# zju3dv/LoG

Measured on AMD Instinct MI355X. Metric: Gaussians/sec fwd+bwd @1080p, higher is better.
Workload: dtype f32; 1 GPU; 30M random Gaussians (seed 0, opacity 0.999), 1920x1080, 8 orbit views/GPU, fwd+bwd; north_star / configs[3] per GPU; gaussians=30000000, width=1920, height=1080, views_per_gpu=8, streams_per_gpu=1, parallelism=single GPU, 1 view(s) in flight per GPU (HIP streams)

## Files before the change

include/lograst.h:

```cpp
#ifndef LOGRAST_H
#define LOGRAST_H

#include <stddef.h>
#include <stdint.h>

#ifdef __cplusplus
extern "C" {
#endif

#define LOGRAST_VERSION 4
#define LOGRAST_TILE 16
#define LOGRAST_REC_FLOATS 16
#define LOGRAST_BWD_ROW_FLOATS 16

#define LOGRAST_FILTER_NONE 0
#define LOGRAST_FORM_AUTO 0
#define LOGRAST_FORM_ROWS 1
#define LOGRAST_FORM_QUADRANT 2
#define LOGRAST_FILTER_DILATE 1
#define LOGRAST_FILTER_CLAMP 2

#define LOGRAST_STATUS_WORDS 8
#define LOGRAST_STATUS_OVERFLOW 0
#define LOGRAST_STATUS_LAST_INSTANCES 1
// ... 102 lines not shown

size_t lograst_sparse_segment_floats(int32_t kmax);
int lograst_pack_rows(const float* rows, int32_t groups, int64_t rows_per_group, int32_t kmax, float* packed,
                      uint32_t* overflow, void* stream);
int lograst_pack_rows_clear(float* rows, int32_t groups, int64_t rows_per_group, int32_t kmax, float* packed,
                            uint32_t* overflow, void* stream);
int lograst_pack_rows_hinted(float* rows, int32_t groups, int64_t rows_per_group, int32_t kmax, float* packed,
                             uint32_t* overflow, int32_t clear, const uint32_t* hint, int64_t hint_rows, void* stream);
int lograst_unpack_rows(float* dest, const float* packed, int32_t segments, int32_t kmax, int64_t rows_per_group,
                        int64_t dest_group_rows, int32_t atomic, void* stream);
int lograst_add_visible(float* seen, const int32_t* radii, int64_t n, void* stream);
int lograst_add_visible_n(float* seen, const int32_t* const* radii, int32_t k, int64_t n, void* stream);

int lograst_knob_count(void);
int lograst_knob_info(int32_t index, const char** name, int32_t* dflt, int32_t* lo, int32_t* hi, const char** what);
int lograst_set_knob(const char* name, int32_t value);
int lograst_get_knob(const char* name, int32_t* value);
int lograst_reset_knobs(void);

int lograst_read_state(const void* tile_state, uint32_t* num_instances_host, uint32_t* overflow_host,
                       uint32_t* max_tile_len_host, uint32_t* rect_instances_host, void* stream);

int lograst_set_tile_cull(int enabled);

#define LOGRAST_BWD_SCRATCH_ZEROED 1
#define LOGRAST_BWD_ACCUMULATE 2
#define LOGRAST_BWD_CONIC_TOUCHED_ONLY 4
#define LOGRAST_BWD_ACCUMULATE_ROWS 8
#define LOGRAST_GRAD_ROW_FLOATS 16

int lograst_backward(const lograst_view* view, int32_t n, const float* means3d, const float* scales,
                     const float* rotations, const int32_t* radii, const void* geom, const void* tile_state,
                     const uint32_t* point_list, const float* final_t, const int32_t* n_contrib,
                     const float* dl_dimage, float* dl_dmeans2d, float* bwd_rows, float* dl_dopacities,
                     float* dl_dcolors, float* dl_dmeans3d, float* dl_dscales, float* dl_drotations,
                     const float* point_weight, int32_t flags, void* stream);

int lograst_backward_aux(const lograst_view* view, int32_t n, const float* means3d, const float* scales,
                         const float* rotations, const int32_t* radii, const void* geom, const void* tile_state,
                         const uint32_t* point_list, const float* final_t, const int32_t* n_contrib,
                         const float* aux_colors, const float* dl_dimage, const float* dl_daux_image, float* dl_dmeans2d,
                         float* bwd_rows, int32_t bwd_row_floats, float* dl_dopacities, float* dl_dcolors,
                         float* dl_daux_colors, float* dl_dmeans3d, float* dl_dscales, float* dl_drotations,
                         const float* point_weight, int32_t flags, void* stream);

int lograst_project_backward(const lograst_view* view, int32_t n, const float* means3d, const float* scales,
// ... 314 lines not shown
```

log_amd/_lib.py:

```python
import ctypes
import os

_HERE = os.path.dirname(os.path.abspath(__file__))
LIB_PATH = os.environ.get("LOGRAST_LIB") or os.path.join(_HERE, "lib", "liblograst.so")

FILTER_NONE, FILTER_DILATE, FILTER_CLAMP = 0, 1, 2
FORM_AUTO, FORM_ROWS, FORM_QUADRANT = 0, 1, 2
GRAD_ROW_FLOATS = 16
REC_FLOATS = 16
BWD_ROW_FLOATS = 16
NUM_KERNELS = 22
NUM_KERNEL_SLOTS = 23

c_void_p, c_int32, c_uint32, c_float, c_size_t = (ctypes.c_void_p, ctypes.c_int32, ctypes.c_uint32,
                                                  ctypes.c_float, ctypes.c_size_t)


class LograstView(ctypes.Structure):
    _fields_ = [
        ("width", c_int32), ("height", c_int32),
        ("tanfovx", c_float), ("tanfovy", c_float),
        ("scale_modifier", c_float),
        ("filter_mode", c_int32), ("ndc_cull", c_int32), ("extras", c_int32),
        ("viewmatrix", c_void_p), ("projmatrix", c_void_p), ("bg", c_void_p),
# ... 92 lines not shown
                            + [c_void_p] * 7 + [c_int32, c_void_p, c_void_p, c_void_p, c_void_p]),
    "lograst_forward_render_aux": (ctypes.c_int, [ctypes.POINTER(LograstView), c_int32, c_void_p, c_void_p, c_void_p,
                                                  c_void_p, c_uint32, c_uint32, c_void_p, c_void_p, c_void_p, c_void_p,
                                                  c_void_p, c_void_p, c_void_p, c_int32, c_void_p, c_void_p, c_void_p,
                                                  c_void_p]),
    "lograst_forward_speculative_aux": (ctypes.c_int, [ctypes.POINTER(LograstView), c_int32] + [c_void_p] * 10
                                        + [c_uint32, c_uint32] + [c_void_p] * 7 + [c_int32, c_void_p, c_void_p, c_void_p]
                                        + [ctypes.POINTER(c_uint32), ctypes.POINTER(c_uint32), c_void_p]),
    "lograst_tile_rows": (ctypes.c_int, [ctypes.POINTER(LograstView), c_int32, c_void_p, c_void_p, c_void_p, c_void_p,
                                         c_void_p]),
    "lograst_stream_copy": (ctypes.c_int, [c_void_p, c_void_p, c_size_t, c_int32, c_void_p]),
    "lograst_sparse_segment_floats": (c_size_t, [c_int32]),
    "lograst_pack_rows": (ctypes.c_int, [c_void_p, c_int32, ctypes.c_int64, c_int32, c_void_p, c_void_p, c_void_p]),
    "lograst_pack_rows_clear": (ctypes.c_int, [c_void_p, c_int32, ctypes.c_int64, c_int32, c_void_p, c_void_p, c_void_p]),
    "lograst_pack_rows_hinted": (ctypes.c_int, [c_void_p, c_int32, ctypes.c_int64, c_int32, c_void_p, c_void_p, c_int32, c_void_p,
                                                ctypes.c_int64, c_void_p]),
    "lograst_add_visible": (ctypes.c_int, [c_void_p, c_void_p, ctypes.c_int64, c_void_p]),
    "lograst_add_visible_n": (ctypes.c_int, [c_void_p, c_void_p, c_int32, ctypes.c_int64, c_void_p]),
    "lograst_unpack_rows": (ctypes.c_int, [c_void_p, c_void_p, c_int32, c_int32, ctypes.c_int64, ctypes.c_int64, c_int32,
                                           c_void_p]),
    "lograst_read_state": (ctypes.c_int, [c_void_p, ctypes.POINTER(c_uint32), ctypes.POINTER(c_uint32),
                                          ctypes.POINTER(c_uint32), ctypes.POINTER(c_uint32), c_void_p]),
    "lograst_set_tile_cull": (ctypes.c_int, [ctypes.c_int]),
    "lograst_knob_count": (ctypes.c_int, []),
    "lograst_knob_info": (ctypes.c_int, [c_int32, ctypes.POINTER(ctypes.c_char_p), ctypes.POINTER(c_int32),
                                         ctypes.POINTER(c_int32), ctypes.POINTER(c_int32), ctypes.POINTER(ctypes.c_char_p)]),
    "lograst_set_knob": (ctypes.c_int, [ctypes.c_char_p, c_int32]),
    "lograst_get_knob": (ctypes.c_int, [ctypes.c_char_p, ctypes.POINTER(c_int32)]),
    "lograst_reset_knobs": (ctypes.c_int, []),
    "lograst_backward": (ctypes.c_int, [ctypes.POINTER(LograstView), c_int32] + [c_void_p] * 18 + [c_int32, c_void_p]),
    "lograst_backward_aux": (ctypes.c_int, [ctypes.POINTER(LograstView), c_int32] + [c_void_p] * 14 + [c_int32]
                             + [c_void_p] * 7 + [c_int32, c_void_p]),
    "lograst_project_backward": (ctypes.c_int, [ctypes.POINTER(LograstView), c_int32] + [c_void_p] * 10),
    "lograst_camera_scratch_bytes": (c_size_t, [c_int32]),
    "lograst_backward_camera": (ctypes.c_int, [ctypes.POINTER(LograstView), c_int32] + [c_void_p] * 18 + [c_int32]
                                + [c_void_p] * 3 + [c_size_t, c_void_p]),
    "lograst_project_backward_camera": (ctypes.c_int, [ctypes.POINTER(LograstView), c_int32] + [c_void_p] * 12
                                        + [c_size_t, c_void_p]),
    "lograst_pose_apply": (ctypes.c_int, [c_int32, c_int32] + [c_void_p] * 7),
    "lograst_pose_backward": (ctypes.c_int, [c_int32, c_int32] + [c_void_p] * 8),
    "lograst_sh_forward": (ctypes.c_int, [c_int32, c_int32, c_int32] + [c_void_p] * 6),
    "lograst_sh_backward": (ctypes.c_int, [c_int32, c_int32, c_int32] + [c_void_p] * 7 + [c_int32, c_void_p]),
    "lograst_knn_scratch_bytes": (c_size_t, [c_int32]),
    "lograst_knn_mean_dist2": (ctypes.c_int, [c_int32, c_void_p, c_void_p, c_void_p, c_size_t, c_void_p]),
    "lograst_lod_scratch_bytes": (c_size_t, [c_int32, c_int32, c_int32]),
    "lograst_lod_traverse": (ctypes.c_int, [c_int32, c_int32, c_int32] + [c_void_p] * 6 + [c_int32, c_void_p, c_void_p,
# ... 125 lines not shown
```

log_amd/csrc/api.hip:

```cpp
#include <hip/hip_runtime.h>

#include <cmath>
#include <cstdint>
#include <cstdio>
#include <cstdlib>
#include <cstring>
#include <mutex>
#include <atomic>
#include <string>
#include <vector>

#include "common.hpp"
#include "launch.hpp"
#include "decide.hpp"

static thread_local std::string g_err;
static int lr_fail(int code, const std::string& msg) {
  g_err = msg;
  return code;
}
#define LR_HIP(expr)                                                                                   \
  do {                                                                                                 \
    hipError_t _e = (expr);                                                                            \
    if (_e != hipSuccess)                                                                              \
// ... 94 lines not shown
}
static bool lr_big_input(int32_t n) { return n >= lr_knob(LRKNOB_HELPER_MIN_N); }
static LrPlan lr_plan(const LrView& v, int32_t n) {
  LrPlan p;
  p.tiles = (uint32_t)v.gx * (uint32_t)v.gy;
  lr_pick_batch(p, n, (uint32_t)v.gx, (uint32_t)v.gy);
  p.batches = p.batch ? ((uint32_t)n + p.batch - 1u) / p.batch : 0u;
  p.band = lr_band_sparse(v, (int)p.batch);
  p.staged_k = lr_fill_staged_k(p);
  p.big_input = lr_big_input(n);
  return p;
}

static std::atomic<int> g_tile_cull{-1};
static int lr_tile_cull() {
  int c = g_tile_cull.load(std::memory_order_relaxed);
  if (c < 0) {
    c = lr_env_int("LOGRAST_TILE_CULL", 1) ? 1 : 0;
    g_tile_cull.store(c, std::memory_order_relaxed);
  }
  return c;
}

static const char* kKernelNames[LOGRAST_NUM_KERNELS] = {
    "compute_radius", "project", "scan_tiles", "fill_keys", "sort_small", "sort_large", "sort_huge",
    "blend_fwd", "blend_bwd", "project_bwd", "knn3", "lod_traverse", "counter_update", "sparse_adam",
    "id_histogram", "gather_activate", "activate_bwd", "count_huge", "rebase_slots", "lazy_tail",
    "loss_fwd", "loss_bwd", "recolor"};
struct ProfRec { int slot; hipEvent_t a, b; bool own_a; };
struct ProfLast { hipStream_t stream; unsigned long long call; hipEvent_t ev; bool valid; };
static thread_local unsigned long long g_prof_call = 0;
static ProfLast g_prof_last = {nullptr, 0, nullptr, false};
static bool g_prof_on = false;
static std::vector<ProfRec> g_prof_open;
static std::vector<ProfRec> g_prof_done;
static std::vector<hipEvent_t> g_event_pool;
static double g_prof_ms[LOGRAST_NUM_KERNELS];
static int64_t g_prof_cnt[LOGRAST_NUM_KERNELS];
static std::mutex g_prof_mu;

static hipEvent_t lr_get_event() {
  if (!g_event_pool.empty()) { hipEvent_t e = g_event_pool.back(); g_event_pool.pop_back(); return e; }
  hipEvent_t e;
  (void)hipEventCreate(&e);
  return e;
}
// ... 584 lines not shown
  if (value < k->lo || value > k->hi) return lr_fail(LOGRAST_ERR_ARG, std::string(name) + ": value out of range");
  std::lock_guard<std::mutex> lk(g_knob_mu);
  g_knob_set[k->id] = true;
  g_knob_over[k->id] = value;
  lr_resolve_knobs_locked();
  return LOGRAST_OK;
}
int lograst_get_knob(const char* name, int32_t* value) {
  const LrKnobInfo* k = lr_find_knob(name);
  if (!k || !value) return lr_fail(LOGRAST_ERR_ARG, "unknown knob or NULL pointer");
  *value = lr_knob(k->id);
  return LOGRAST_OK;
}
int lograst_reset_knobs(void) {
  std::lock_guard<std::mutex> lk(g_knob_mu);
  for (bool& set : g_knob_set) set = false;
  lr_resolve_knobs_locked();
  return LOGRAST_OK;
}

int lograst_set_tile_cull(int enabled) {
  const int old = lr_tile_cull();
  g_tile_cull.store(enabled ? 1 : 0, std::memory_order_relaxed);
  return old;
}

int lograst_read_state(const void* tile_state, uint32_t* num_instances_host, uint32_t* overflow_host,
                       uint32_t* max_tile_len_host, uint32_t* rect_instances_host, void* stream) {
  if (!tile_state) return lr_fail(LOGRAST_ERR_ARG, "tile_state is NULL");
  uint32_t hdr[8] = {0, 0, 0, 0, 0, 0, 0, 0};
  hipStream_t s = (hipStream_t)stream;
  LR_HIP(hipMemcpyAsync(hdr, tile_state, sizeof(hdr), hipMemcpyDeviceToHost, s));
  LR_HIP(hipStreamSynchronize(s));
  if (num_instances_host) *num_instances_host = hdr[LR_HDR_NUM];
  if (overflow_host) *overflow_host = hdr[LR_HDR_OVERFLOW];
  if (max_tile_len_host) *max_tile_len_host = hdr[LR_HDR_MAXLEN];
  if (rect_instances_host) *rect_instances_host = hdr[LR_HDR_RECT];
  return LOGRAST_OK;
}

struct LrBackwardAux { int on; const float* aux_colors; const float* dl_daux_image; int32_t bwd_row_floats; float* dl_daux_colors; };
struct LrBackwardCam { int on; float* dl_dview; float* dl_dproj; void* scratch; size_t scratch_bytes; };
static int lr_check_camera(const LrView& v, int32_t n, int32_t flags, const LrBackwardCam& cam, hipStream_t s, bool* done) {
  *done = false;
  if (!cam.dl_dview || !cam.dl_dproj) return lr_fail(LOGRAST_ERR_ARG, "dl_dviewmatrix / dl_dprojmatrix are NULL");
  if (flags & (LOGRAST_BWD_ACCUMULATE | LOGRAST_BWD_ACCUMULATE_ROWS))
// ... 1181 lines not shown
```

log_amd/csrc/blend.hip:

```cpp
#include "common.hpp"
#include "launch.hpp"
#define LR_LANDED(q0, q1, c, i)                                                                                  \
  asm volatile("" : "+v"((q0).x), "+v"((q0).y), "+v"((q0).z), "+v"((q0).w), "+v"((q1).x), "+v"((q1).y), "+v"((q1).z), \
               "+v"((q1).w), "+v"(c), "+v"(i))

LR_DEV uint32_t lr_tile_of_block(uint32_t b, uint32_t tiles, int gx, int gy, int mode,
                                 const uint32_t* __restrict__ state) {
  if (mode == 3) return b < tiles ? state[lr_order_off(tiles) + b] : 0xffffffffu;
  if (mode == 1) {
    uint32_t nper = (tiles + 7u) >> 3;
    uint32_t t = (b & 7u) * nper + (b >> 3);
    return t < tiles ? t : 0xffffffffu;
  }
  if (mode == 2) {
    uint32_t nsbx = ((uint32_t)gx + 3u) >> 2, nsby = ((uint32_t)gy + 3u) >> 2;
    uint32_t r = b >> 3, sb = (r >> 4) * 8u + (b & 7u), local = r & 15u;
    if (sb >= nsbx * nsby) return 0xffffffffu;
    uint32_t tx = (sb % nsbx) * 4u + (local & 3u), ty = (sb / nsbx) * 4u + (local >> 2);
    if (tx >= (uint32_t)gx || ty >= (uint32_t)gy) return 0xffffffffu;
    return ty * (uint32_t)gx + tx;
  }
  return b < tiles ? b : 0xffffffffu;
}
static inline __host__ __device__ uint32_t lr_blend_grid(uint32_t tiles, int gx, int gy, int mode) {
// ... 527 lines not shown
  return lr_bank_select<0xc>(a + lr_dpp_perm<0x140>(a), b + lr_dpp_perm<0x140>(b));
}
LR_DEV float lr_row_pair4(float p, float q) {
  return lr_bank_select<0xa>(p + lr_dpp_perm<0x141>(p), q + lr_dpp_perm<0x141>(q));
}
LR_DEV float lr_quad_total(float x) {
  x = x + lr_dpp_perm<0xB1>(x);
  return x + lr_dpp_perm<0x4E>(x);
}

LR_DEV void lr_atomic_add_noret(float* p, float x) {
  asm volatile("global_atomic_add_f32 %0, %1, off" : : "v"(p), "v"(x) : "memory");
}

LR_DEV uint32_t lr_take_bit(uint64_t& m) {
  const uint32_t j = min((uint32_t)(__ffsll((long long)m) - 1), 64u);
  m &= m - 1ull;
  return j;
}
LR_DEV uint64_t lr_row_mask(int row, uint64_t m0, uint64_t m1, uint64_t m2, uint64_t m3) {
  return row == 0 ? m0 : (row == 1 ? m1 : (row == 2 ? m2 : m3));
}

template <bool MASKS>
__global__ void __launch_bounds__(256)
lr_blend_bwd_rows_kernel(LrView v, const float4* __restrict__ geom, const uint32_t* __restrict__ state,
                         uint32_t tiles, const uint32_t* __restrict__ plist, uint32_t capacity,
                         const float* __restrict__ final_T, const int* __restrict__ n_contrib,
                         const float* __restrict__ dL_dimage, float* __restrict__ acc_rows,
                         int xcd_mode, int block_test, const uint64_t* __restrict__ masks) {
  __shared__ float4 lr_stage[4][65 * LR_RB_SLOT];
  if (lr_bail(state, capacity)) return;
  const uint32_t tile = lr_tile_of_block(blockIdx.x, tiles, v.gx, v.gy, xcd_mode, state);
  if (tile >= tiles) return;
  const uint32_t* offsets = state + lr_offsets_off(tiles);
  const uint32_t beg = offsets[tile];
  const int lane = threadIdx.x & 63, wq = threadIdx.x >> 6;
  constexpr bool use_masks = MASKS;
  const bool masks_ok = use_masks && lr_masks_usable(v, state, tiles, LR_MASK_FORM_ROWS);
  const int row = lane >> 4, li = lane & 15;
  const int tx = tile % (uint32_t)v.gx, ty = tile / (uint32_t)v.gx;
  const int qx0 = tx * 16 + (wq & 1) * 8, qy0 = ty * 16 + (wq >> 1) * 8;
  const int px = qx0 + (row & 1) * 4 + (li & 3), py = qy0 + (row >> 1) * 4 + (li >> 2);
  const float pxf = (float)px, pyf = (float)py;
  const bool in = (px < v.W) && (py < v.H);
  const size_t plane = (size_t)v.W * v.H;
  const size_t pix = in ? (size_t)py * v.W + px : 0;
  const float sx = 0.5f * (float)v.W, sy = 0.5f * (float)v.H;
  const float Tf = in ? final_T[pix] : 0.f;
  const int lastc = in ? n_contrib[pix] : 0;
  const float dp0 = in ? dL_dimage[pix] : 0.f;
  const float dp1 = in ? dL_dimage[plane + pix] : 0.f;
  const float dp2 = in ? dL_dimage[2 * plane + pix] : 0.f;
  const float bgdot = lr_fma(v.bg[0], dp0, lr_fma(v.bg[1], dp1, v.bg[2] * dp2));
  float T = Tf, acc0 = 0.f, acc1 = 0.f, acc2 = 0.f;
  int rmax = lastc;
#pragma unroll
  for (int off = 8; off > 0; off >>= 1) rmax = max(rmax, __shfl_xor(rmax, off));
  const int rm0 = lr_readlane_i(rmax, 0), rm1 = lr_readlane_i(rmax, 16), rm2 = lr_readlane_i(rmax, 32),
            rm3 = lr_readlane_i(rmax, 48);
  const int maxc = max(max(rm0, rm1), max(rm2, rm3));
  if (maxc == 0) return;

  float* const sf = reinterpret_cast<float*>(lr_stage[wq]);
#define LR_SF(f, j) sf[(f) * 65 + (j)]
  const uint32_t sf_lds = (uint32_t)(uintptr_t)(__attribute__((address_space(3))) float*)sf;
  if (lane < 10) LR_SF(lane, 64) = lane == 9 ? __uint_as_float(0xffffffffu) : 0.f;

  const int qd = li >> 2, sel = li & 3;
  const int slot = sel == 0 ? (qd == 0 ? 6 : (qd == 1 ? 8 : (qd == 2 ? 7 : 5)))
                            : (sel == 1 ? (qd == 0 ? 0 : (qd == 1 ? 2 : (qd == 2 ? 1 : 3))) : 4);
  const bool on_a = sel < 2 || li == 2, on_b = sel < 2 || li == 10;
  float* const dst = acc_rows + slot;

  const float bx[2] = {(float)qx0, (float)(qx0 + 4)}, by[2] = {(float)qy0, (float)(qy0 + 4)};

  const int top = use_masks ? ((maxc + 63) & ~63) : maxc;
  const uint32_t nchunks = ((uint32_t)top + 63u) >> 6;
  auto load_id = [&](uint32_t c) -> uint32_t {
    const int pos = top - 1 - (int)(c * 64u) - lane;
    const bool ok = c < nchunks && pos >= 0 && pos < maxc;
    const uint32_t got = plist[beg + (ok ? (uint32_t)pos : 0u)];
    return ok ? got : 0xffffffffu;
  };
  const uint4* const mbase = !use_masks ? nullptr : !masks_ok ? reinterpret_cast<const uint4*>(state)
                             : reinterpret_cast<const uint4*>(masks + 16 * lr_mask_slot(beg, tile) +
                                                              4 * __builtin_amdgcn_readfirstlane(wq));
  const size_t mstride = masks_ok ? 8u : 0u;
  const uint64_t mfill = masks_ok ? 0ull : ~0ull;
  struct Masks4 { uint64_t m0, m1, m2, m3; };
  auto load_masks = [&](uint32_t c) -> Masks4 {
    if (!use_masks) return Masks4{0ull, 0ull, 0ull, 0ull};
    const uint32_t cf = ((uint32_t)top >> 6) - 1u - min(c, nchunks - 1u);
    const uint4* mp = mbase + mstride * (size_t)cf;
    const uint4 lo = mp[0], hi4 = mp[1];
    return Masks4{(((uint64_t)lo.y << 32) | lo.x) | mfill, (((uint64_t)lo.w << 32) | lo.z) | mfill,
                  (((uint64_t)hi4.y << 32) | hi4.x) | mfill, (((uint64_t)hi4.w << 32) | hi4.z) | mfill};
  };
  auto wanted = [&](const Masks4& m) -> bool {
    return !use_masks || (((m.m0 | m.m1 | m.m2 | m.m3) >> (63 - lane)) & 1ull) != 0ull;
  };
  auto gather = [&](uint32_t idv, bool want, float4& q0, float4& q1, float& qc) {
    const float4* rp = geom + LR_REC_QUADS * (size_t)(want ? idv : 0u);
    q0 = rp[0]; q1 = rp[1]; qc = reinterpret_cast<const float*>(rp)[8];
  };
  uint32_t id_n = load_id(0), id_nn = load_id(1);
  Masks4 mk_n = load_masks(0), mk_nn = load_masks(1);
  float4 g0_n, g1_n;
  float cb_n;
  gather(id_n, id_n != 0xffffffffu && wanted(mk_n), g0_n, g1_n, cb_n);
  LR_LANDED(g0_n, g1_n, cb_n, id_nn);

  for (uint32_t ch = 0; ch < nchunks; ch++) {
    const int hi = top - (int)(ch * 64u);
    const uint32_t id = id_n;
    const float4 g0 = g0_n, g1 = g1_n;
    const float cb = cb_n;
    const Masks4 mk = mk_n;
    id_n = id_nn;
    mk_n = mk_nn;
    gather(id_n, id_n != 0xffffffffu && wanted(mk_n), g0_n, g1_n, cb_n);
    id_nn = load_id(ch + 2);
    mk_nn = load_masks(ch + 2);
    __builtin_amdgcn_fence(__ATOMIC_RELEASE, "wavefront");
    __builtin_amdgcn_wave_barrier();
    if (id != 0xffffffffu && wanted(mk)) {
      LR_SF(0, lane) = g0.x; LR_SF(1, lane) = g0.y; LR_SF(2, lane) = g0.z; LR_SF(3, lane) = g0.w;
      LR_SF(4, lane) = g1.x; LR_SF(5, lane) = g1.y; LR_SF(6, lane) = g1.z; LR_SF(7, lane) = g1.w;
      LR_SF(8, lane) = cb; LR_SF(9, lane) = __uint_as_float(id);
    }
    __builtin_amdgcn_fence(__ATOMIC_RELEASE, "wavefront");
    __builtin_amdgcn_wave_barrier();
    __builtin_amdgcn_fence(__ATOMIC_ACQUIRE, "wavefront");
    const bool valid = id != 0xffffffffu;
    const int pos = hi - 1 - lane;
    bool r0 = valid & (pos < rm0), r1 = valid & (pos < rm1), r2 = valid & (pos < rm2), r3 = valid & (pos < rm3);
    if (!use_masks) {
      const LrSupport sp = lr_support_prepare(g0.x, g0.y, g0.z, g0.w, g1.x, g1.y);
      if (block_test) {
        bool k0, k1, k2, k3;
        const lr_f2 X0 = {bx[0], bx[1]}, X1 = {bx[0] + 3.f, bx[1] + 3.f};
        lr_support_box2(sp, X0, X1, lr_f2{by[0], by[0]}, lr_f2{by[0] + 3.f, by[0] + 3.f}, k0, k1);
        lr_support_box2(sp, X0, X1, lr_f2{by[1], by[1]}, lr_f2{by[1] + 3.f, by[1] + 3.f}, k2, k3);
        r0 = r0 && k0; r1 = r1 && k1; r2 = r2 && k2; r3 = r3 && k3;
      } else {
        const bool q = lr_support_box(sp, bx[0], bx[0] + 7.f, by[0], by[0] + 7.f);
        const bool bb = sp.mode == 2;
        const bool x_lo = !bb || (sp.mx - sp.ex <= bx[0] + 3.f), x_hi = !bb || (sp.mx + sp.ex >= bx[1]);
        const bool y_lo = !bb || (sp.my - sp.ey <= by[0] + 3.f), y_hi = !bb || (sp.my + sp.ey >= by[1]);
        r0 = r0 && q && x_lo && y_lo;
        r1 = r1 && q && x_hi && y_lo;
        r2 = r2 && q && x_lo && y_hi;
        r3 = r3 && q && x_hi && y_hi;
      }
    }
    uint64_t mrow;
    if (use_masks) mrow = lr_mask_before(lr_row_mask(row, __builtin_bitreverse64(mk.m0), __builtin_bitreverse64(mk.m1),
                                                     __builtin_bitreverse64(mk.m2), __builtin_bitreverse64(mk.m3)), hi, rmax);
    else mrow = lr_row_mask(row, __ballot(r0), __ballot(r1), __ballot(r2), __ballot(r3));
    while (__builtin_amdgcn_ballot_w64(mrow != 0ull) != 0) {
      const uint32_t ja = lr_take_bit(mrow), jb = lr_take_bit(mrow);
      float fa[10], fb[10];
      {
        const uint32_t aa = sf_lds + 4u * ja, ab = sf_lds + 4u * jb;
        asm volatile(
            "ds_read_b32 %0, %20\n ds_read_b32 %10, %21\n"
            "ds_read_b32 %1, %20 offset:260\n ds_read_b32 %11, %21 offset:260\n"
            "ds_read_b32 %2, %20 offset:520\n ds_read_b32 %12, %21 offset:520\n"
            "ds_read_b32 %3, %20 offset:780\n ds_read_b32 %13, %21 offset:780\n"
            "ds_read_b32 %4, %20 offset:1040\n ds_read_b32 %14, %21 offset:1040\n"
            "ds_read_b32 %5, %20 offset:1300\n ds_read_b32 %15, %21 offset:1300\n"
            "ds_read_b32 %6, %20 offset:1560\n ds_read_b32 %16, %21 offset:1560\n"
            "ds_read_b32 %7, %20 offset:1820\n ds_read_b32 %17, %21 offset:1820\n"
            "ds_read_b32 %8, %20 offset:2080\n ds_read_b32 %18, %21 offset:2080\n"
            "ds_read_b32 %9, %20 offset:2340\n ds_read_b32 %19, %21 offset:2340\n"
            "s_waitcnt lgkmcnt(0)"
            : "=&v"(fa[0]), "=&v"(fa[1]), "=&v"(fa[2]), "=&v"(fa[3]), "=&v"(fa[4]), "=&v"(fa[5]), "=&v"(fa[6]), "=&v"(fa[7]),
              "=&v"(fa[8]), "=&v"(fa[9]), "=&v"(fb[0]), "=&v"(fb[1]), "=&v"(fb[2]), "=&v"(fb[3]), "=&v"(fb[4]), "=&v"(fb[5]),
              "=&v"(fb[6]), "=&v"(fb[7]), "=&v"(fb[8]), "=&v"(fb[9])
            : "v"(aa), "v"(ab)
            : "memory");
      }
      const lr_f2 Ar = {fa[2], fb[2]}, Br = {fa[3], fb[3]}, Cr = {fa[4], fb[4]};
      const lr_f2 op2 = {fa[5], fb[5]};
      const lr_f2 cr = {fa[6], fb[6]}, cg = {fa[7], fb[7]}, cbl = {fa[8], fb[8]};
      const uint32_t gida = __float_as_uint(fa[9]), gidb = __float_as_uint(fb[9]);
      const lr_f2 dx2 = lr_f2{fa[0], fb[0]} - pxf, dy2 = lr_f2{fa[1], fb[1]} - pyf;
      const lr_f2 hdx2 = dx2 * -0.5f, hdy2 = dy2 * -0.5f;
      const lr_f2 bdx = Br * dx2;
      const lr_f2 pw2 = lr_fma2(Ar * dx2, hdx2, lr_fma2(Cr * dy2, hdy2, lr_f2{-bdx.x, -bdx.y} * dy2));
      const lr_f2 G2 = lr_exp2(pw2);
      const lr_f2 al2 = op2 * G2;
      const float alpha0 = fminf(0.99f, al2.x), alpha1 = fminf(0.99f, al2.y);
      const int k0 = hi - 1 - (int)ja, k1 = hi - 1 - (int)jb;
      const bool hit0 = (k0 < lastc) & !(pw2.x > 0.f) & !(alpha0 < 1.0f / 255.0f);
      const bool hit1 = (k1 < lastc) & !(pw2.y > 0.f) & !(alpha1 < 1.0f / 255.0f);
      const lr_f2 alpha = {hit0 ? alpha0 : 0.f, hit1 ? alpha1 : 0.f};
      const bool any = __builtin_amdgcn_ballot_w64((alpha.x > 0.f) | (alpha.y > 0.f)) != 0;
      if (!any) continue;
      const lr_f2 G = {hit0 ? G2.x : 0.f, hit1 ? G2.y : 0.f};
      const lr_f2 om = 1.f - alpha;
      lr_f2 rc = {__builtin_amdgcn_rcpf(om.x), __builtin_amdgcn_rcpf(om.y)};
      rc = lr_fma2(lr_fma2(-om, rc, lr_f2{1.f, 1.f}), rc, rc);
      const float Ta = T * rc.x, Tb = Ta * rc.y;
      const lr_f2 T2 = {Ta, Tb};
      T = Tb;
      const lr_f2 w = alpha * T2;
      const float a0r = lr_fma(alpha.x, cr.x, om.x * acc0), a0g = lr_fma(alpha.x, cg.x, om.x * acc1),
                  a0b = lr_fma(alpha.x, cbl.x, om.x * acc2);
      lr_f2 dL_dalpha = lr_fma2(cr - lr_f2{acc0, a0r}, lr_f2{dp0, dp0},
                                lr_fma2(cg - lr_f2{acc1, a0g}, lr_f2{dp1, dp1}, (cbl - lr_f2{acc2, a0b}) * dp2));
      dL_dalpha = lr_fma2(dL_dalpha, T2, -(Tf * rc) * bgdot);
      acc0 = lr_fma(alpha.y, cr.y, om.y * a0r);
      acc1 = lr_fma(alpha.y, cg.y, om.y * a0g);
      acc2 = lr_fma(alpha.y, cbl.y, om.y * a0b);
      const lr_f2 dL_dG = op2 * dL_dalpha;
      const lr_f2 gdx = G * dx2, gdy = G * dy2;
      const lr_f2 dG_ddx = lr_fma2(-Ar, gdx, -(Br * gdy));
      const lr_f2 dG_ddy = lr_fma2(-Cr, gdy, -(Br * gdx));
      const lr_f2 c0 = w * dp0, c1 = w * dp1, c2 = w * dp2, go = G * dL_dalpha;
      const lr_f2 mxs = dL_dG * dG_ddx * sx, mys = dL_dG * dG_ddy * sy;
      const lr_f2 kA = -0.5f * gdx * dx2 * dL_dG, kB = -gdx * dy2 * dL_dG, kC = -0.5f * gdy * dy2 * dL_dG;
      const float s1a = lr_quad_total(lr_row_pair4(lr_row_pair8(c0.x, c1.x), lr_row_pair8(c2.x, go.x)));
      const float s1b = lr_quad_total(lr_row_pair4(lr_row_pair8(c0.y, c1.y), lr_row_pair8(c2.y, go.y)));
      const float s2a = lr_quad_total(lr_row_pair4(lr_row_pair8(mxs.x, mys.x), lr_row_pair8(kA.x, kB.x)));
      const float s2b = lr_quad_total(lr_row_pair4(lr_row_pair8(mxs.y, mys.y), lr_row_pair8(kA.y, kB.y)));
      float s3 = lr_row_pair8(kC.x, kC.y);
      s3 = lr_quad_total(s3 + lr_dpp_perm<0x141>(s3));
      const float xa = sel == 0 ? s1a : (sel == 1 ? s2a : s3);
      const float xb = sel == 0 ? s1b : (sel == 1 ? s2b : s3);
      if (on_a && gida != 0xffffffffu) lr_atomic_add_noret(dst + (size_t)gida * LOGRAST_BWD_ROW_FLOATS, xa);
      if (on_b && gidb != 0xffffffffu) lr_atomic_add_noret(dst + (size_t)gidb * LOGRAST_BWD_ROW_FLOATS, xb);
    }
  }
}

template <bool EXTRAS>
__global__ void __launch_bounds__(256) __attribute__((amdgpu_waves_per_eu(5)))
lr_blend_fwd_rows_kernel(LrView v, const float4* __restrict__ geom, const uint32_t* __restrict__ state,
                         uint32_t tiles, const uint32_t* __restrict__ plist, uint32_t capacity,
                         float* __restrict__ image, float* __restrict__ final_T, int* __restrict__ n_contrib,
                         int* __restrict__ pid, float* __restrict__ pwp, float* __restrict__ pw,
                         float4* __restrict__ zero_rows, int xcd_mode, int cull, uint32_t* __restrict__ lazy_state,
                         int lazy, uint64_t* __restrict__ masks, uint32_t* __restrict__ hdr_w, int block_test,
                         int exact_masks) {
  __shared__ float4 lr_stage[4][65 * LR_RB_SLOT];
  if (lr_bail(state, capacity)) return;
  if (lazy == 2 && !lazy_state[LR_HDR_OPEN]) return;
  if (masks && blockIdx.x == 0 && threadIdx.x == 0) hdr_w[LR_HDR_MASKS] = LR_MASK_FORM_ROWS;
  const uint32_t tile = lr_tile_of_block(blockIdx.x, tiles, v.gx, v.gy, xcd_mode, state);
  if (tile >= tiles) return;
  const uint32_t* offsets = state + lr_offsets_off(tiles);
  uint32_t beg = offsets[tile];
  uint32_t end = offsets[tile + 1], first;
  bool clamped;
  const int lane = threadIdx.x & 63, wq = threadIdx.x >> 6;
  __shared__ uint64_t lr_mbuf[4][LR_MBUF_CHUNKS * 4];
// ... 239 lines not shown
      hipLaunchKernelGGL(lr_blend_fwd_kernel<false>, dim3(grid), dim3(256), 0, s, v, g4, state, tiles, plist, capacity,
                         image, final_T, n_contrib, pid, pwp, pw, z4, xcd_mode, 1, lazy_state, lazy, masks, hdr_w, nullptr, nullptr);
  }
  if (lazy != 2) lr_prof_end(LRK_BLEND_FWD, s);
}

void lr_launch_blend_bwd(const LrView& v, const void* geom, const uint32_t* state, uint32_t tiles,
                         const uint32_t* plist, uint32_t capacity, const float* final_T, const int* n_contrib,
                         const float* dL_dimage, float* acc_rows, int big_input, const uint64_t* masks, hipStream_t s,
                         const float* aux_colors, const float* dL_daux) {
  const int xcd_mode = lr_knob(LRKNOB_XCD_MODE);
  uint32_t grid = lr_blend_grid(tiles, v.gx, v.gy, xcd_mode);
  const int rows = !aux_colors && lr_blend_bwd_form(v, big_input) == (int)LR_MASK_FORM_ROWS;
  const int block_test = lr_knob(LRKNOB_BWD_BLOCK_TEST);
  lr_prof_begin(LRK_BLEND_BWD, s);
  const bool use_masks = masks != nullptr && v.mask_form == (rows ? (int)LR_MASK_FORM_ROWS : (int)LR_MASK_FORM_QUAD);
  const float4* g4 = reinterpret_cast<const float4*>(geom);
  if (aux_colors && use_masks)
    hipLaunchKernelGGL((lr_blend_bwd_kernel<true, true>), dim3(grid), dim3(256), 0, s, v, g4, state, tiles, plist, capacity,
                       final_T, n_contrib, dL_dimage, acc_rows, xcd_mode, masks, aux_colors, dL_daux);
  else if (aux_colors)
    hipLaunchKernelGGL((lr_blend_bwd_kernel<false, true>), dim3(grid), dim3(256), 0, s, v, g4, state, tiles, plist, capacity,
                       final_T, n_contrib, dL_dimage, acc_rows, xcd_mode, masks, aux_colors, dL_daux);
  else if (rows && use_masks)
    hipLaunchKernelGGL(lr_blend_bwd_rows_kernel<true>, dim3(grid), dim3(256), 0, s, v, g4, state, tiles, plist, capacity,
                       final_T, n_contrib, dL_dimage, acc_rows, xcd_mode, block_test, masks);
  else if (rows)
    hipLaunchKernelGGL(lr_blend_bwd_rows_kernel<false>, dim3(grid), dim3(256), 0, s, v, g4, state, tiles, plist, capacity,
                       final_T, n_contrib, dL_dimage, acc_rows, xcd_mode, block_test, masks);
  else if (use_masks)
    hipLaunchKernelGGL(lr_blend_bwd_kernel<true>, dim3(grid), dim3(256), 0, s, v, g4, state, tiles, plist, capacity,
                       final_T, n_contrib, dL_dimage, acc_rows, xcd_mode, masks, nullptr, nullptr);
  else
    hipLaunchKernelGGL(lr_blend_bwd_kernel<false>, dim3(grid), dim3(256), 0, s, v, g4, state, tiles, plist, capacity,
                       final_T, n_contrib, dL_dimage, acc_rows, xcd_mode, masks, nullptr, nullptr);
  lr_prof_end(LRK_BLEND_BWD, s);
}
```

log_amd/csrc/common.hpp:

```cpp
#pragma once
#include <hip/hip_runtime.h>
#include <stdint.h>
#include <atomic>

#include "../../include/lograst.h"

#define LR_WAVE 64
#define LR_TILE 16

#define LR_CTR_STRIDE 16
#define LR_RANKED_TILES 4
#define LR_HDR_WORDS 16
#define LR_HDR_NUM 0
#define LR_HDR_OVERFLOW 1
#define LR_HDR_MAXLEN 2
#define LR_HDR_BATCH 6
#define LR_HDR_CULL 5
#define LR_HDR_RECT 4
#define LR_HDR_SPARSE 3
#define LR_HDR_SPAN 8
#define LR_HDR_HUGE 7
#define LR_HDR_LAZY 9
#define LR_HDR_KEYS_LO 11
#define LR_HDR_KEYS_HI 12
// ... 451 lines not shown
  const float* mask; const float* fg;
  int64_t ms[3], fs[3];
  const float* bg;
  float* gt_out;
};

enum LrKernelSlot {
  LRK_RADIUS = 0, LRK_PROJECT, LRK_SCAN, LRK_FILL, LRK_SORT_SMALL, LRK_SORT_LARGE, LRK_SORT_HUGE,
  LRK_BLEND_FWD, LRK_BLEND_BWD, LRK_PROJECT_BWD, LRK_MISC, LRK_LOD, LRK_COUNTER, LRK_ADAM, LRK_HIST, LRK_GATHER, LRK_GATHER_BWD, LRK_RESERVED,
  LRK_REBASE, LRK_LAZY_TAIL,
  LRK_LOSS_FWD, LRK_LOSS_BWD,
  LRK_RECOLOR
};
void lr_prof_begin(int slot, hipStream_t s);
void lr_prof_end(int slot, hipStream_t s);
enum LrKnob {
  LRKNOB_HELPER_MIN_N, LRKNOB_HIT_MASKS, LRKNOB_LAZY_SORT, LRKNOB_PBWD_LIST, LRKNOB_MID_RANK, LRKNOB_MID_COOP,
  LRKNOB_DEFER_TILES, LRKNOB_HUGE_CHUNK, LRKNOB_BATCH_PLANES, LRKNOB_BATCH_SLOTS, LRKNOB_SEPARATE_ZERO,
  LRKNOB_FILL_XCD_ORDER, LRKNOB_FILL_NT, LRKNOB_XCD_MODE, LRKNOB_PROJECT_BLOCKS, LRKNOB_BWD_ROWS, LRKNOB_FWD_ROWS,
  LRKNOB_FILL_STAGED, LRKNOB_FILL_PER_THREAD, LRKNOB_BAND_SPARSE, LRKNOB_FWD_BLOCK_TEST, LRKNOB_BWD_BLOCK_TEST,
  LRKNOB_COUNT
};
int lr_knob(LrKnob k);
```

log_amd/rasterizer.py:

```python
import contextlib
import ctypes
import math
import threading
from typing import NamedTuple

import torch
import torch.nn as nn

from . import _lib


class GaussianRasterizationSettings(NamedTuple):
    image_height: int
    image_width: int
    tanfovx: float
    tanfovy: float
    bg: torch.Tensor
    scale_modifier: float
    viewmatrix: torch.Tensor
    projmatrix: torch.Tensor
    sh_degree: int
    campos: torch.Tensor
    prefiltered: bool
    debug: bool
# ... 213 lines not shown
    if st is None:
        return 0, False, 0, 0
    w = st.cpu().tolist()
    return int(w[1]), bool(w[2]), int(w[3]), int(w[4])


def last_overflow(device=None):
    n, o = last_state_info(device)[:2]
    return n, o


def overflow_since_reset(device=None, reset=True):
    st = _status.get(device if device is not None else _current_device())
    if st is None:
        return dict(overflowed=False, max_instances=0, max_tile_len=0, forwards=0)
    w = st.cpu().tolist()
    if reset:
        st.zero_()
    return dict(overflowed=bool(w[0]), max_instances=int(w[5]), max_tile_len=int(w[6]), forwards=int(w[7]))


def set_tile_cull(enabled):
    return bool(_lib.lib().lograst_set_tile_cull(1 if enabled else 0))


def _stream_ptr(device):
    return ctypes.c_void_p(torch.cuda.current_stream(device).cuda_stream)


def _ptr(t):
    return ctypes.c_void_p(t.data_ptr()) if t is not None and t.numel() > 0 else ctypes.c_void_p(0)


def _dev_f32(t, device):
    return t.detach().to(device=device, dtype=torch.float32).contiguous()


def _knob(name):
    val = ctypes.c_int32(0)
    _lib.lib().lograst_get_knob(name, ctypes.byref(val))
    return val.value


TILE = 16


# ... 1090 lines not shown
```

Measured before the change: 10.55 billion Gaussians/s.

## Stage per-row backward gradient sums in LDS and commit them per chunk

In the row-form blend backward kernel, per-Gaussian partial sums from each pixel row are written to an LDS scratch area instead of being atomically added to global memory right away. A commit routine then adds up the four row contributions per Gaussian and issues one global atomic per field. That commit is deferred to overlap with the next gather and runs mid-batch when more than 32 Gaussians are touched. The goal is to cut global atomic traffic, at the cost of extra LDS, wave barriers and a lower waves-per-EU occupancy hint. It is enabled by default through an environment/API toggle.

```diff
diff --git a/include/lograst.h b/include/lograst.h
--- a/include/lograst.h
+++ b/include/lograst.h
@@ -148,6 +148,8 @@
                        uint32_t* max_tile_len_host, uint32_t* rect_instances_host, void* stream);
 
 int lograst_set_tile_cull(int enabled);
+
+int lograst_set_bwd_chunk_commits(int enabled);
 
 #define LOGRAST_BWD_SCRATCH_ZEROED 1
 #define LOGRAST_BWD_ACCUMULATE 2
diff --git a/log_amd/_lib.py b/log_amd/_lib.py
--- a/log_amd/_lib.py
+++ b/log_amd/_lib.py
@@ -138,6 +138,7 @@
     "lograst_read_state": (ctypes.c_int, [c_void_p, ctypes.POINTER(c_uint32), ctypes.POINTER(c_uint32),
                                           ctypes.POINTER(c_uint32), ctypes.POINTER(c_uint32), c_void_p]),
     "lograst_set_tile_cull": (ctypes.c_int, [ctypes.c_int]),
+    "lograst_set_bwd_chunk_commits": (ctypes.c_int, [ctypes.c_int]),
     "lograst_knob_count": (ctypes.c_int, []),
     "lograst_knob_info": (ctypes.c_int, [c_int32, ctypes.POINTER(ctypes.c_char_p), ctypes.POINTER(c_int32),
                                          ctypes.POINTER(c_int32), ctypes.POINTER(c_int32), ctypes.POINTER(ctypes.c_char_p)]),
diff --git a/log_amd/csrc/api.hip b/log_amd/csrc/api.hip
--- a/log_amd/csrc/api.hip
+++ b/log_amd/csrc/api.hip
@@ -140,6 +140,16 @@
   return c;
 }
 
+static std::atomic<int> g_bwd_chunk_commits{-1};
+int lr_bwd_chunk_commits() {
+  int c = g_bwd_chunk_commits.load(std::memory_order_relaxed);
+  if (c < 0) {
+    c = lr_env_int("LOGRAST_BWD_CHUNK_COMMITS", 1) ? 1 : 0;
+    g_bwd_chunk_commits.store(c, std::memory_order_relaxed);
+  }
+  return c;
+}
+
 static const char* kKernelNames[LOGRAST_NUM_KERNELS] = {
     "compute_radius", "project", "scan_tiles", "fill_keys", "sort_small", "sort_large", "sort_huge",
     "blend_fwd", "blend_bwd", "project_bwd", "knn3", "lod_traverse", "counter_update", "sparse_adam",
@@ -770,6 +780,12 @@
 int lograst_set_tile_cull(int enabled) {
   const int old = lr_tile_cull();
   g_tile_cull.store(enabled ? 1 : 0, std::memory_order_relaxed);
+  return old;
+}
+
+int lograst_set_bwd_chunk_commits(int enabled) {
+  const int old = lr_bwd_chunk_commits();
+  g_bwd_chunk_commits.store(enabled ? 1 : 0, std::memory_order_relaxed);
   return old;
 }
 
diff --git a/log_amd/csrc/blend.hip b/log_amd/csrc/blend.hip
--- a/log_amd/csrc/blend.hip
+++ b/log_amd/csrc/blend.hip
@@ -573,14 +573,42 @@
   return row == 0 ? m0 : (row == 1 ? m1 : (row == 2 ? m2 : m3));
 }
 
-template <bool MASKS>
-__global__ void __launch_bounds__(256)
+#define LR_CC_SLOTS 32u
+#define LR_CC_ROW (9u * LR_CC_SLOTS)
+#define LR_CC_WAVE (4u * LR_CC_ROW)
+LR_DEV void lr_bwd_commit_chunk(const float* sf, const float* sums, int lane, uint32_t base, uint32_t cnt,
+                                float* __restrict__ acc_rows) {
+  __builtin_amdgcn_fence(__ATOMIC_RELEASE, "wavefront");
+  __builtin_amdgcn_wave_barrier();
+  __builtin_amdgcn_fence(__ATOMIC_ACQUIRE, "wavefront");
+  asm volatile("" : "+v"(lane));
+  const uint32_t e = (uint32_t)lane / 9u, f = (uint32_t)lane - 9u * e;
+  for (uint32_t n0 = 0; n0 < cnt; n0 += 7u) {
+    const uint32_t n = n0 + e;
+    if (lane < 63 && n < cnt) {
+      const uint32_t gid = __float_as_uint(sf[9 * 65 + base + n]);
+      const uint32_t w = __float_as_uint(sf[11 * 65 + base + n]);
+      const float* cell = sums + 9u * n0 + (uint32_t)lane;
+      const float t0 = cell[0], t1 = cell[LR_CC_ROW], t2 = cell[2 * LR_CC_ROW], t3 = cell[3 * LR_CC_ROW];
+      float sum = 0.f;
+      sum = (w & 1u) ? sum + t0 : sum;
+      sum = (w & 2u) ? sum + t1 : sum;
+      sum = (w & 4u) ? sum + t2 : sum;
+      sum = (w & 8u) ? sum + t3 : sum;
+      lr_atomic_add_noret(acc_rows + (size_t)gid * LOGRAST_BWD_ROW_FLOATS + f, sum);
+    }
+  }
+}
+
+template <bool MASKS, bool CHUNK>
+__global__ void __launch_bounds__(256) __attribute__((amdgpu_waves_per_eu(MASKS ? 5 : 4)))
 lr_blend_bwd_rows_kernel(LrView v, const float4* __restrict__ geom, const uint32_t* __restrict__ state,
                          uint32_t tiles, const uint32_t* __restrict__ plist, uint32_t capacity,
                          const float* __restrict__ final_T, const int* __restrict__ n_contrib,
                          const float* __restrict__ dL_dimage, float* __restrict__ acc_rows,
                          int xcd_mode, int block_test, const uint64_t* __restrict__ masks) {
   __shared__ float4 lr_stage[4][65 * LR_RB_SLOT];
+  __shared__ float lr_sums[CHUNK ? 4 * LR_CC_WAVE : 1];
   if (lr_bail(state, capacity)) return;
   const uint32_t tile = lr_tile_of_block(blockIdx.x, tiles, v.gx, v.gy, xcd_mode, state);
   if (tile >= tiles) return;
@@ -616,13 +644,16 @@
   float* const sf = reinterpret_cast<float*>(lr_stage[wq]);
 #define LR_SF(f, j) sf[(f) * 65 + (j)]
   const uint32_t sf_lds = (uint32_t)(uintptr_t)(__attribute__((address_space(3))) float*)sf;
-  if (lane < 10) LR_SF(lane, 64) = lane == 9 ? __uint_as_float(0xffffffffu) : 0.f;
+  if (lane < 11) LR_SF(lane, 64) = lane == 9 ? __uint_as_float(0xffffffffu) : 0.f;
 
   const int qd = li >> 2, sel = li & 3;
   const int slot = sel == 0 ? (qd == 0 ? 6 : (qd == 1 ? 8 : (qd == 2 ? 7 : 5)))
                             : (sel == 1 ? (qd == 0 ? 0 : (qd == 1 ? 2 : (qd == 2 ? 1 : 3))) : 4);
   const bool on_a = sel < 2 || li == 2, on_b = sel < 2 || li == 10;
   float* const dst = acc_rows + slot;
+  float* const wsums = lr_sums + (CHUNK ? LR_CC_WAVE * (uint32_t)wq : 0u);
+  char* const cell = reinterpret_cast<char*>(wsums + (CHUNK ? LR_CC_ROW * (uint32_t)row + (uint32_t)slot : 0u));
+  uint32_t pend_base = 0u, pend_cnt = 0u;
 
   const float bx[2] = {(float)qx0, (float)(qx0 + 4)}, by[2] = {(float)qy0, (float)(qy0 + 4)};
 
@@ -668,6 +699,7 @@
     const float4 g0 = g0_n, g1 = g1_n;
     const float cb = cb_n;
     const Masks4 mk = mk_n;
+    if (CHUNK) lr_bwd_commit_chunk(sf, wsums, lane, pend_base, pend_cnt, acc_rows);
     id_n = id_nn;
     mk_n = mk_nn;
     gather(id_n, id_n != 0xffffffffu && wanted(mk_n), g0_n, g1_n, cb_n);
@@ -675,14 +707,13 @@
     mk_nn = load_masks(ch + 2);
     __builtin_amdgcn_fence(__ATOMIC_RELEASE, "wavefront");
     __builtin_amdgcn_wave_barrier();
-    if (id != 0xffffffffu && wanted(mk)) {
+    const bool staged = id != 0xffffffffu && wanted(mk);
+    if (staged) {
       LR_SF(0, lane) = g0.x; LR_SF(1, lane) = g0.y; LR_SF(2, lane) = g0.z; LR_SF(3, lane) = g0.w;
       LR_SF(4, lane) = g1.x; LR_SF(5, lane) = g1.y; LR_SF(6, lane) = g1.z; LR_SF(7, lane) = g1.w;
-      LR_SF(8, lane) = cb; LR_SF(9, lane) = __uint_as_float(id);
-    }
-    __builtin_amdgcn_fence(__ATOMIC_RELEASE, "wavefront");
-    __builtin_amdgcn_wave_barrier();
-    __builtin_amdgcn_fence(__ATOMIC_ACQUIRE, "wavefront");
+      LR_SF(8, lane) = cb;
+      if (!CHUNK) LR_SF(9, lane) = __uint_as_float(id);
+    }
     const bool valid = id != 0xffffffffu;
     const int pos = hi - 1 - lane;
     bool r0 = valid & (pos < rm0), r1 = valid & (pos < rm1), r2 = valid & (pos < rm2), r3 = valid & (pos < rm3);
@@ -705,11 +736,50 @@
         r3 = r3 && q && x_hi && y_hi;
       }
     }
-    uint64_t mrow;
-    if (use_masks) mrow = lr_mask_before(lr_row_mask(row, __builtin_bitreverse64(mk.m0), __builtin_bitreverse64(mk.m1),
-                                                     __builtin_bitreverse64(mk.m2), __builtin_bitreverse64(mk.m3)), hi, rmax);
-    else mrow = lr_row_mask(row, __ballot(r0), __ballot(r1), __ballot(r2), __ballot(r3));
-    while (__builtin_amdgcn_ballot_w64(mrow != 0ull) != 0) {
+    uint64_t v0, v1, v2, v3;
+    if (use_masks) {
+      v0 = lr_mask_before(__builtin_bitreverse64(mk.m0), hi, rm0); v1 = lr_mask_before(__builtin_bitreverse64(mk.m1), hi, rm1);
+      v2 = lr_mask_before(__builtin_bitreverse64(mk.m2), hi, rm2); v3 = lr_mask_before(__builtin_bitreverse64(mk.m3), hi, rm3);
+    } else {
+      v0 = __ballot(r0); v1 = __ballot(r1); v2 = __ballot(r2); v3 = __ballot(r3);
+    }
+    uint32_t ulo = 0u, uhi = 0u;
+    bool split = false;
+    if (CHUNK) {
+      if (use_masks) {
+        const uint64_t st = __ballot(staged);
+        v0 &= st; v1 &= st; v2 &= st; v3 &= st;
+      }
+      const uint64_t u = v0 | v1 | v2 | v3;
+      ulo = (uint32_t)u; uhi = (uint32_t)(u >> 32);
+      split = __popcll(u) > (int)LR_CC_SLOTS;
+      const bool upper = split && lane >= 32;
+      const uint32_t c = __builtin_amdgcn_mbcnt_hi(uhi, __builtin_amdgcn_mbcnt_lo(upper ? 0u : ulo, 0u));
+      if ((u >> lane) & 1ull) {
+        const uint32_t nib = (uint32_t)((v0 >> lane) & 1ull) | ((uint32_t)((v1 >> lane) & 1ull) << 1) |
+                             ((uint32_t)((v2 >> lane) & 1ull) << 2) | ((uint32_t)((v3 >> lane) & 1ull) << 3);
+        const uint32_t at = (upper ? LR_CC_SLOTS : 0u) + c;
+        LR_SF(10, lane) = __uint_as_float(36u * c);
+        LR_SF(9, at) = __uint_as_float(id);
+        LR_SF(11, at) = __uint_as_float(nib);
+      }
+    }
+    __builtin_amdgcn_fence(__ATOMIC_RELEASE, "wavefront");
+    __builtin_amdgcn_wave_barrier();
+    __builtin_amdgcn_fence(__ATOMIC_ACQUIRE, "wavefront");
+    const uint64_t ph0 = split ? 0xffffffffull : ~0ull;
+    uint64_t mrow = lr_row_mask(row, v0 & ph0, v1 & ph0, v2 & ph0, v3 & ph0);
+    auto more = [&]() -> bool {
+      if (__builtin_amdgcn_ballot_w64(mrow != 0ull) != 0) return true;
+      if (!(CHUNK && split)) return false;
+      split = false;
+      lr_bwd_commit_chunk(sf, wsums, lane, 0u, (uint32_t)__popc(ulo), acc_rows);
+      ulo = 0u;
+      mrow = lr_row_mask(row, v0 & ~ph0, v1 & ~ph0, v2 & ~ph0, v3 & ~ph0);
+      return true;
+    };
+    const uint32_t pend_split = split ? LR_CC_SLOTS : 0u;
+    while (more()) {
       const uint32_t ja = lr_take_bit(mrow), jb = lr_take_bit(mrow);
       float fa[10], fb[10];
       {
@@ -724,18 +794,22 @@
             "ds_read_b32 %6, %20 offset:1560\n ds_read_b32 %16, %21 offset:1560\n"
             "ds_read_b32 %7, %20 offset:1820\n ds_read_b32 %17, %21 offset:1820\n"
             "ds_read_b32 %8, %20 offset:2080\n ds_read_b32 %18, %21 offset:2080\n"
-            "ds_read_b32 %9, %20 offset:2340\n ds_read_b32 %19, %21 offset:2340\n"
+            "ds_read_b32 %9, %20 offset:%22\n ds_read_b32 %19, %21 offset:%22\n"
             "s_waitcnt lgkmcnt(0)"
             : "=&v"(fa[0]), "=&v"(fa[1]), "=&v"(fa[2]), "=&v"(fa[3]), "=&v"(fa[4]), "=&v"(fa[5]), "=&v"(fa[6]), "=&v"(fa[7]),
               "=&v"(fa[8]), "=&v"(fa[9]), "=&v"(fb[0]), "=&v"(fb[1]), "=&v"(fb[2]), "=&v"(fb[3]), "=&v"(fb[4]), "=&v"(fb[5]),
               "=&v"(fb[6]), "=&v"(fb[7]), "=&v"(fb[8]), "=&v"(fb[9])
-            : "v"(aa), "v"(ab)
+            : "v"(aa), "v"(ab), "n"(CHUNK ? 4 * 65 * 10 : 4 * 65 * 9)
             : "memory");
       }
       const lr_f2 Ar = {fa[2], fb[2]}, Br = {fa[3], fb[3]}, Cr = {fa[4], fb[4]};
       const lr_f2 op2 = {fa[5], fb[5]};
       const lr_f2 cr = {fa[6], fb[6]}, cg = {fa[7], fb[7]}, cbl = {fa[8], fb[8]};
       const uint32_t gida = __float_as_uint(fa[9]), gidb = __float_as_uint(fb[9]);
+      auto stage_sums = [&](float xa, float xb) {
+        if (on_a && ja != 64u) *reinterpret_cast<float*>(cell + gida) = xa;
+        if (on_b && jb != 64u) *reinterpret_cast<float*>(cell + gidb) = xb;
+      };
       const lr_f2 dx2 = lr_f2{fa[0], fb[0]} - pxf, dy2 = lr_f2{fa[1], fb[1]} - pyf;
       const lr_f2 hdx2 = dx2 * -0.5f, hdy2 = dy2 * -0.5f;
       const lr_f2 bdx = Br * dx2;
@@ -748,7 +822,10 @@
       const bool hit1 = (k1 < lastc) & !(pw2.y > 0.f) & !(alpha1 < 1.0f / 255.0f);
       const lr_f2 alpha = {hit0 ? alpha0 : 0.f, hit1 ? alpha1 : 0.f};
       const bool any = __builtin_amdgcn_ballot_w64((alpha.x > 0.f) | (alpha.y > 0.f)) != 0;
-      if (!any) continue;
+      if (!any) {
+        if (CHUNK) stage_sums(0.f, 0.f);
+        continue;
+      }
       const lr_f2 G = {hit0 ? G2.x : 0.f, hit1 ? G2.y : 0.f};
       const lr_f2 om = 1.f - alpha;
       lr_f2 rc = {__builtin_amdgcn_rcpf(om.x), __builtin_amdgcn_rcpf(om.y)};
@@ -780,10 +857,19 @@
       s3 = lr_quad_total(s3 + lr_dpp_perm<0x141>(s3));
       const float xa = sel == 0 ? s1a : (sel == 1 ? s2a : s3);
       const float xb = sel == 0 ? s1b : (sel == 1 ? s2b : s3);
-      if (on_a && gida != 0xffffffffu) lr_atomic_add_noret(dst + (size_t)gida * LOGRAST_BWD_ROW_FLOATS, xa);
-      if (on_b && gidb != 0xffffffffu) lr_atomic_add_noret(dst + (size_t)gidb * LOGRAST_BWD_ROW_FLOATS, xb);
-    }
-  }
+      if (CHUNK) {
+        stage_sums(xa, xb);
+      } else {
+        if (on_a && gida != 0xffffffffu) lr_atomic_add_noret(dst + (size_t)gida * LOGRAST_BWD_ROW_FLOATS, xa);
+        if (on_b && gidb != 0xffffffffu) lr_atomic_add_noret(dst + (size_t)gidb * LOGRAST_BWD_ROW_FLOATS, xb);
+      }
+    }
+    if (CHUNK) {
+      pend_base = pend_split;
+      pend_cnt = (uint32_t)__popc(ulo) + (uint32_t)__popc(uhi);
+    }
+  }
+  if (CHUNK) lr_bwd_commit_chunk(sf, wsums, lane, pend_base, pend_cnt, acc_rows);
 }
 
 template <bool EXTRAS>
@@ -1069,12 +1155,12 @@
   else if (aux_colors)
     hipLaunchKernelGGL((lr_blend_bwd_kernel<false, true>), dim3(grid), dim3(256), 0, s, v, g4, state, tiles, plist, capacity,
                        final_T, n_contrib, dL_dimage, acc_rows, xcd_mode, masks, aux_colors, dL_daux);
-  else if (rows && use_masks)
-    hipLaunchKernelGGL(lr_blend_bwd_rows_kernel<true>, dim3(grid), dim3(256), 0, s, v, g4, state, tiles, plist, capacity,
+  else if (rows) {
+    auto kernel = lr_bwd_chunk_commits() ? (use_masks ? lr_blend_bwd_rows_kernel<true, true> : lr_blend_bwd_rows_kernel<false, true>)
+                                         : (use_masks ? lr_blend_bwd_rows_kernel<true, false> : lr_blend_bwd_rows_kernel<false, false>);
+    hipLaunchKernelGGL(kernel, dim3(grid), dim3(256), 0, s, v, g4, state, tiles, plist, capacity,
                        final_T, n_contrib, dL_dimage, acc_rows, xcd_mode, block_test, masks);
-  else if (rows)
-    hipLaunchKernelGGL(lr_blend_bwd_rows_kernel<false>, dim3(grid), dim3(256), 0, s, v, g4, state, tiles, plist, capacity,
-                       final_T, n_contrib, dL_dimage, acc_rows, xcd_mode, block_test, masks);
+  }
   else if (use_masks)
     hipLaunchKernelGGL(lr_blend_bwd_kernel<true>, dim3(grid), dim3(256), 0, s, v, g4, state, tiles, plist, capacity,
                        final_T, n_contrib, dL_dimage, acc_rows, xcd_mode, masks, nullptr, nullptr);
diff --git a/log_amd/csrc/common.hpp b/log_amd/csrc/common.hpp
--- a/log_amd/csrc/common.hpp
+++ b/log_amd/csrc/common.hpp
@@ -497,3 +497,4 @@
   LRKNOB_COUNT
 };
 int lr_knob(LrKnob k);
+int lr_bwd_chunk_commits();
diff --git a/log_amd/rasterizer.py b/log_amd/rasterizer.py
--- a/log_amd/rasterizer.py
+++ b/log_amd/rasterizer.py
@@ -259,6 +259,10 @@
 
 def set_tile_cull(enabled):
     return bool(_lib.lib().lograst_set_tile_cull(1 if enabled else 0))
+
+
+def set_bwd_chunk_commits(enabled):
+    return bool(_lib.lib().lograst_set_bwd_chunk_commits(1 if enabled else 0))
 
 
 def _stream_ptr(device):
```

Measured after the change: 10.57 billion Gaussians/s (median of 5 runs). Within noise of the previous version (+0.2%).
